# Jiraiya812/Fast-CU-Decision-HEVC

Measured on NVIDIA B200. Metric: cu_decision_ctus_per_s_1080p_all_intra, higher is better.
Workload: dtype int32

## Files before the change

### fast-cu-decision-hevc_b200/csrc/capi.cu

```cuda
#include <cuda_runtime.h>
#include <algorithm>
#include <chrono>
#include <cstdio>
#include <cstdlib>
#include <cstring>
#include "handle.h"
#include "rmd_tc2.cuh"
#include "rmd_tc3.cuh"
#include "tcm_host.h"

using namespace cucd;

static_assert(kPackedCtuBytes == CUCD_PACKED_CTU_BYTES && kPackedU16Off == CUCD_PACKED_U16_OFFSET && kPackedB13Off == CUCD_PACKED_B13_OFFSET,
              "kernel-side packed cost layout must match include/cucudecide.h");

namespace cucd {
std::string g_createError;

bool pin_host_range(cucd_handle* h, const void* ptr, size_t bytes) {
  if (!ptr || !bytes) return false;
  uintptr_t lo = (uintptr_t)ptr, hi = lo + bytes;
  for (const auto& r : h->pins) if (r.first <= lo && hi <= r.second) return true;
  cudaPointerAttributes at;
  if (cudaPointerGetAttributes(&at, ptr) == cudaSuccess && at.type == cudaMemoryTypeHost) {
// ... 24 lines not shown
                              int recStride, uint32_t* out, uint8_t* outPacked, const uint8_t* needed = nullptr) {
  FrameSource fs;
  fs.org = org; fs.rec = rec; fs.orgPicStride = orgPic; fs.recPicStride = recPic; fs.orgStride = orgStride; fs.recStride = recStride;
  fs.W = h->cfg.width; fs.H = h->cfg.height; fs.ctusPerRow = h->ctusPerRow; fs.ctusPerPic = h->ctusPerPic; fs.out = out; fs.outPacked = outPacked; fs.needed = needed;
  return fs;
}
FeaturePlanes make_feature_planes(const cucd_handle* h, const int16_t* org, long long orgPic, int orgStride) {
  FeaturePlanes fp;
  fp.org = org; fp.orgPicStride = orgPic; fp.orgStride = orgStride; fp.W = h->cfg.width; fp.H = h->cfg.height;
  fp.ctusPerRow = h->ctusPerRow; fp.ctusPerPic = h->ctusPerPic; fp.bitDepth = h->cfg.bit_depth;
  return fp;
}

cudaError_t launch_rmd_auto(cucd_handle* h, const FrameSource& fs, int nPics, cudaStream_t st) {
  if (h->useTensor == 1 && h->cfg.bit_depth == 8)
    return launch_rmd_frames_tc2(fs, nPics, h->cfg.strong_intra_smoothing, h->dTc2Tables.p, h->dTc2Tables.p + tc2::kWinTableBytes, h->dHadamard.p, st, &h->launches);
  if (h->useTensor >= 1)
    return launch_rmd_frames_tc3(fs, nPics, h->cfg.bit_depth, h->cfg.strong_intra_smoothing, h->dTc3Tables.p, h->dTc3Tables.p + tc3::kWinTableBytes16,
                                 h->dTc3Tables.p + tc3::kWinTableBytes16 + tc3::kN4TableBytes16, st, &h->launches);
  return launch_rmd_frames(fs, nPics, h->cfg.bit_depth, h->cfg.strong_intra_smoothing, st, &h->launches);
}

bool plane_ok(const void* p, long long picStride, int stride, int width) {
  return ((uintptr_t)p & 15) == 0 && (stride & 7) == 0 && (picStride & 7) == 0 && stride >= width;
}

void fit_batch(cucd_handle* h, int nPics, const uint32_t* hist, int32_t* thr, double* yc ) {
  const int nBlocks = (h->cfg.width / 4) * (h->cfg.height / 4);
  h->pool.run(nPics * 15, [=](int i) {
    const int p = i / 15, f = 1 + i % 15;
    const double y = tcm_fit_one(hist + ((size_t)p * kHistFreqs + f) * kHistBins, nBlocks);
// ... 79 lines not shown
  ok = ok && cudaEventCreate(&h->evK0) == cudaSuccess && cudaEventCreate(&h->evK1) == cudaSuccess;
  ok = ok && cudaEventCreateWithFlags(&h->evMask, cudaEventDisableTiming) == cudaSuccess;
  ok = ok && cudaEventCreateWithFlags(&h->evDevUp, cudaEventDisableTiming) == cudaSuccess && cudaEventCreateWithFlags(&h->evDevDone, cudaEventDisableTiming) == cudaSuccess;
  for (int i = 0; i < cucd_handle::kTimeRing; i++) ok = ok && cudaEventCreate(&h->evRmd0[i]) == cudaSuccess && cudaEventCreate(&h->evRmd1[i]) == cudaSuccess;
  for (FrameSlot& s : h->slots) {
    ok = ok && cudaEventCreateWithFlags(&s.evHist, cudaEventDisableTiming) == cudaSuccess &&
         cudaEventCreateWithFlags(&s.evFork, cudaEventDisableTiming) == cudaSuccess &&
         cudaEventCreateWithFlags(&s.evJoin, cudaEventDisableTiming) == cudaSuccess;
    ok = ok && s.dHist.reserve(P * kHistFreqs * kHistBins) == cudaSuccess && s.dThr.reserve(P * kHistFreqs) == cudaSuccess;
    ok = ok && s.hHist.reserve(P * kHistFreqs * kHistBins) == cudaSuccess && s.hThr.reserve(P * kHistFreqs) == cudaSuccess;
  }
  ok = ok && h->dObf.reserve(P * (size_t)(cfg->width / 4) * (cfg->height / 4)) == cudaSuccess;
  ok = ok && h->dOutlier.reserve(P * (size_t)cfg->width * cfg->height) == cudaSuccess;
  for (int d = 0; d < 4; d++) ok = ok && h->dNum[d].reserve(P * std::max<size_t>(1, h->cuCount[d])) == cudaSuccess && h->dSum[d].reserve(P * std::max<size_t>(1, h->cuCount[d])) == cudaSuccess;
  ok = ok && h->dCtuHad.reserve(P * h->ctusPerPic) == cudaSuccess;
  ok = ok && h->dHadamard.reserve(16384) == cudaSuccess && launch_hadamard_operands(h->dHadamard.p, h->sMain) == cudaSuccess &&
       cudaStreamSynchronize(h->sMain) == cudaSuccess;
  if (ok) {
    std::vector<uint8_t> tab(tc2::kWinTableBytes + tc2::kN4TableBytes);
    tc2::fill_win_tables(tab.data()); tc2::fill_n4_tables(tab.data() + tc2::kWinTableBytes);
    ok = h->dTc2Tables.reserve(tab.size()) == cudaSuccess && cudaMemcpy(h->dTc2Tables.p, tab.data(), tab.size(), cudaMemcpyHostToDevice) == cudaSuccess;
  }
  if (ok) {
    std::vector<uint8_t> tab(tc3::kWinTableBytes16 + tc3::kN4TableBytes16 + tc3::kHadBytes16);
    tc3::fill_win_tables16(tab.data()); tc3::fill_n4_tables16(tab.data() + tc3::kWinTableBytes16);
    tc3::fill_had_tables16(tab.data() + tc3::kWinTableBytes16 + tc3::kN4TableBytes16);
    ok = h->dTc3Tables.reserve(tab.size()) == cudaSuccess && cudaMemcpy(h->dTc3Tables.p, tab.data(), tab.size(), cudaMemcpyHostToDevice) == cudaSuccess;
  }
  h->useTensor = 1;
  { const char* ev = getenv("CUCD_RMD_PATH"); if (ev && !strcmp(ev, "alu")) h->useTensor = 0; }
  if (!ok) {
    const std::string msg = std::string("cucd_create: allocation failed: ") + cudaGetErrorString(cudaGetLastError());
    cucd_destroy(h);
    return fail(nullptr, CUCD_ERR_NOMEM, msg);
  }
  *out = h;
  return CUCD_OK;
}

int cucd_destroy(cucd_handle* h) {
  if (!h) return CUCD_OK;
  cudaSetDevice(h->cfg.device);
  cudaDeviceSynchronize();
  h->pool.stop();
  for (const auto& r : h->pins) cudaHostUnregister((void*)r.first);
  h->dOrg.release(); h->dRec.release(); h->dOrg8.release(); h->dRec8.release(); h->dObf.release(); h->dOutlier.release(); h->dObf8.release(); h->dOutlier8.release();
  h->dCost.release(); h->dCostPacked.release();
  for (FrameSlot& s : h->slots) {
    s.dHist.release(); s.hHist.release(); s.dThr.release(); s.hThr.release();
    if (s.evHist) cudaEventDestroy(s.evHist);
    if (s.evFork) cudaEventDestroy(s.evFork);
    if (s.evJoin) cudaEventDestroy(s.evJoin);
  }
  for (int d = 0; d < 4; d++) { h->dNum[d].release(); h->dSum[d].release(); }
  h->dCtuHad.release(); h->dHadamard.release(); h->dTc2Tables.release();
  h->bOut.release(); h->bStage.release(); h->hStage.release(); h->hStageOut.release(); h->hScratch.release();
  for (auto& r : h->refs) r.buf.release();
  h->dCur.release(); h->dRefPtr.release(); h->dRefStride.release();
  for (int i = 0; i < cucd_handle::kTimeRing; i++) { if (h->evRmd0[i]) cudaEventDestroy(h->evRmd0[i]); if (h->evRmd1[i]) cudaEventDestroy(h->evRmd1[i]); }
  for (int i = 0; i < cucd_handle::kGroups; i++) { if (h->evUpG[i]) cudaEventDestroy(h->evUpG[i]); if (h->evRmdG[i]) cudaEventDestroy(h->evRmdG[i]); }
  h->hDevScratch.release(); h->dDevStage.release();
  if (h->evDevUp) cudaEventDestroy(h->evDevUp);
  if (h->evDevDone) cudaEventDestroy(h->evDevDone);
  h->dNeeded.release();
  if (h->evMask) cudaEventDestroy(h->evMask);
  if (h->evDirect) cudaEventDestroy(h->evDirect);
  if (h->evK0) cudaEventDestroy(h->evK0);
  if (h->evK1) cudaEventDestroy(h->evK1);
  if (h->sUp) cudaStreamDestroy(h->sUp);
  if (h->evUp) cudaEventDestroy(h->evUp);
// ... 389 lines not shown
```

### fast-cu-decision-hevc_b200/csrc/handle.h

```cpp
#pragma once
#include <cuda_runtime.h>
#include <atomic>
#include <condition_variable>
#include <functional>
#include <mutex>
#include <string>
#include <thread>
#include <vector>
#include "../../include/cucudecide.h"
#include "kernels.h"

namespace cucd {

template <class T> struct DevBuf {
  T* p = nullptr; size_t n = 0;
  cudaError_t reserve(size_t count) {
    if (count <= n) return cudaSuccess;
    if (p) cudaFree(p);
    p = nullptr; n = 0;
    cudaError_t e = cudaMalloc(&p, count * sizeof(T));
    if (e == cudaSuccess) n = count;
    return e;
  }
  void release() { if (p) cudaFree(p); p = nullptr; n = 0; }
// ... 95 lines not shown
  long long rmdCalls = 0;
  int launches = 0;
  long long launchTotal = 0;
  std::string err;
  cucd::HostPool pool;
  cucd::FrameSlot slots[2];
  long long begun = 0, ended = 0;
  cucd::DevBuf<int16_t> dOrg, dRec, dObf, dOutlier;
  cucd::DevBuf<uint8_t> dOrg8, dRec8;
  cucd::DevBuf<uint8_t> dObf8, dOutlier8;
  cucd::DevBuf<uint32_t> dCost;
  cucd::DevBuf<uint8_t> dCostPacked;
  cucd::DevBuf<int8_t> dHadamard;
  cucd::DevBuf<uint8_t> dTc3Tables;
  cucd::DevBuf<uint8_t> dTc2Tables;
  int useTensor = 0;
  cucd::DevBuf<int32_t> dNum[4], dSum[4], dCtuHad;
  size_t cuCount[4] = {0, 0, 0, 0};
  bool prune = false; cucd::PruneSwitches sw = {};
  cucd::DevBuf<uint8_t> dNeeded;
  cudaEvent_t evMask = nullptr;
  std::vector<std::pair<uintptr_t, uintptr_t>> pins;
  cucd::DevBuf<uint8_t> bStage; cucd::DevBuf<uint32_t> bOut;
  cucd::PinBuf<uint8_t> hStage, hStageOut, hScratch;
  cudaEvent_t evDirect = nullptr;
  std::vector<int32_t> tmpOffA, tmpOffB;
  std::vector<cucd::RefPlane> refs;
  bool refTableDirty = true;
  cucd::DevBuf<int16_t> dCur; int curStride = 0; bool curSet = false;
  cucd::DevBuf<const int16_t*> dRefPtr; cucd::DevBuf<int32_t> dRefStride;
// ... 27 lines not shown
```

### fast-cu-decision-hevc_b200/csrc/kernels.h

```cpp
#pragma once
#include <cuda_runtime.h>
#include <stdint.h>
#include "rmd_chunk.cuh"

namespace cucd {

constexpr int kHistBins = 4096;
constexpr int kHistFreqs = 16;

cudaError_t launch_rmd_frames(const FrameSource& fs, int nPics, int bitDepth, int strong, cudaStream_t st, int* launches);
cudaError_t configure_rmd_kernels();
cudaError_t configure_rmd_tc2_kernels();
cudaError_t launch_hadamard_operands(int8_t* dst, cudaStream_t st);
cudaError_t launch_rmd_frames_tc2(const FrameSource& fs, int nPics, int strong, const uint8_t* tabWin, const uint8_t* tabN4, const int8_t* hadamard,
                                  cudaStream_t st, int* launches);
int rmd_tc2_smem_bytes();
cudaError_t configure_rmd_tc3_kernels();
cudaError_t launch_rmd_frames_tc3(const FrameSource& fs, int nPics, int bitDepth, int strong, const uint8_t* tabWin16, const uint8_t* tabN416,
                                  const uint8_t* hadamard16, cudaStream_t st, int* launches);
int rmd_tc3_smem_bytes();
cudaError_t launch_rmd_batch_tc2(int log2n, const BatchSource& bs, int strong, const uint8_t* tabWin, const uint8_t* tabN4, const int8_t* hadamard,
                                 cudaStream_t st, int* launches);
cudaError_t launch_rmd_batch(int log2n, const BatchSource& bs, int bitDepth, int strong, cudaStream_t st, int* launches);

struct FeaturePlanes {
  const int16_t* org; long long orgPicStride; int orgStride;
  int W, H, ctusPerRow, ctusPerPic, bitDepth;
};
cudaError_t launch_feature_hist(const FeaturePlanes& fp, int nPics, uint32_t* hist, cudaStream_t st, int* launches);
cudaError_t launch_copy_words(const uint32_t* src, uint32_t* dst, size_t nWords, cudaStream_t st, int* launches);
// ... 63 lines not shown
```

### fast-cu-decision-hevc_b200/csrc/rmd_tc2_kernels.cu

```cuda
#include <cuda_runtime.h>
#include "rmd_tc2.cuh"
#include "rmd_tc_frame.cuh"
#include "satd_tc.cuh"
#include "kernels.h"

namespace cucd {

extern __shared__ __align__(128) unsigned char smem2[];

using namespace tc;
using namespace tc2;
using namespace tcf;

#ifdef CUCD_TC2_TIMING
__device__ long long* g_tc2Dbg = nullptr;
#ifndef CUCD_TC2_STAMP_TID
#define CUCD_TC2_STAMP_TID 0
#endif
#define TC2_STAMP(i) do { if (g_tc2Dbg && threadIdx.x == CUCD_TC2_STAMP_TID) g_tc2Dbg[(size_t)blockIdx.x * 64 + (i)] = clock64(); } while (0)
#define TC2_FINE(i) do { if (g_tc2Dbg && threadIdx.x == CUCD_TC2_STAMP_TID && pass == 0 && (am == 4 || am == -4)) g_tc2Dbg[(size_t)blockIdx.x * 64 + (am == 4 ? 30 : 40) + (i)] = clock64(); } while (0)
#else
#define TC2_STAMP(i) do { } while (0)
#define TC2_FINE(i) do { } while (0)
#endif
#ifdef CUCD_TC2_WARPSKEW
__device__ long long* g_tc2Skew = nullptr;
#define TC2_SKEW(e) do { if (g_tc2Skew && pass == 0 && (am == 4 || (am == 3 && (e) < 2)) && (threadIdx.x & 31) == 0 && threadIdx.x < 128) g_tc2Skew[(size_t)blockIdx.x * 64 + (threadIdx.x >> 5) * 16 + (am == 4 ? (e) : 9 + (e))] = clock64(); } while (0)
#else
#define TC2_SKEW(e) do { } while (0)
#endif

namespace {

struct Tc2Args {
  FrameSource fs;
  BatchSource bs;
  int strong, totalCtus;
  const uint8_t* tabWin; const uint8_t* tabN4; const int8_t* had;
};

constexpr int kIssuerThreads = 32 * kGroups;
constexpr int kCtaThreads = kThreads + kIssuerThreads;
__device__ __forceinline__ void worker_bar() { asm volatile("bar.sync 1, 256;\n" ::: "memory"); }
template <int LOG2N, bool FRAME>
// ... 25 lines not shown
    return;
  }
#pragma unroll
  for (int c = 0; c < C::CTUS; c++) {
    const int cg = unit * C::CTUS + c;
    uint8_t* valid = smem + C::VALID_OFF + c * 256;
    if (ctuX[c] < 0) {
      for (int p = tid; p < C::PUS; p += kThreads) valid[p] = kPuOutside;
      continue;
    }
    const uint8_t* need = ctu_needed<LOG2N>(fs, cg);
    for (int p = tid; p < C::PUS; p += kThreads) valid[p] = pu_state<LOG2N>(fs, need, ctuX[c], ctuY[c], p);
  }
#pragma unroll
  for (int c = 0; c < C::CTUS; c++)
    if (ctuX[c] >= 0) tile_store<Cfg, LOG2N>(tid, fs.W, fs.H, ctuX[c], ctuY[c], tl[c], smem + C::TILE_OFF + c * C::TILE_BYTES);
  worker_bar();
  TC2_STAMP(51);
#pragma unroll
  for (int c = 0; c < C::CTUS; c++)
    if (ctuX[c] >= 0) build_unfiltered<LOG2N>(tid, c, fs.W, fs.H, ctuX[c], ctuY[c], smem + C::TILE_OFF + c * C::TILE_BYTES, smem);
  TC2_STAMP(52);
  if (C::HAS_FILT) {
    worker_bar();
    TC2_STAMP(53);
#pragma unroll
    for (int c = 0; c < C::CTUS; c++)
      if (ctuX[c] >= 0) build_filtered<LOG2N>(tid, c, a.strong, smem);
  }
}

template <int LOG2N, bool FRAME>
__device__ __forceinline__ void tc2_pass(const Tc2Args& a, const int unit, const int pass, const uint32_t tmemBase, uint32_t& ph1, uint32_t& ph2, const Vec16* pre) {
  typedef Cfg<LOG2N> C;
  constexpr int N = C::N, SEG = RowSeg<LOG2N>::value;
  unsigned char* smem = smem2;
  const int tid = threadIdx.x, grp = tid >> 7, rowTid = tid & 127, warp = tid >> 5, lane = tid & 31;
  const Row r = row_map<LOG2N>(tid, pass);
  unsigned char* store = smem + C::STORE_OFF;
  unsigned char* sA1 = smem + C::A1_OFF + grp * 8192;
  unsigned char* sAorg = smem + C::AORG_OFF + grp * 8192;
  uint64_t* mbar1 = reinterpret_cast<uint64_t*>(smem + C::BAR_OFF) + grp;
  uint64_t* mbar2 = mbar1 + kGroups;
  uint64_t* arrA = mbar1 + 2 * kGroups;
  uint64_t* arrB = mbar1 + 3 * kGroups;
  uint32_t* acc = reinterpret_cast<uint32_t*>(smem + C::ACC_OFF);
  const FrameSource& fs = a.fs;
  const int cg = unit * C::CTUS + r.ctu;
  const bool ok = smem[C::VALID_OFF + r.ctu * 256 + (LOG2N == 2 ? 4 * r.pu : r.pu)] == kPuEvaluate;
  const int slot = pu_slot2<LOG2N>(r.ctu, r.pu);

  uint32_t p[16];
  if (ok) {
    uint32_t raw[16];
    if (FRAME) {
      if (pre && pass == 0) {
#pragma unroll
// ... 181 lines not shown
    TC2_SKEW(6);
    if (lateWindow) stage_window(am - 1, angleNext, buf ^ 1);
    if (am > -8) issue_mma1();
    TC2_FINE(7);
    TC2_SKEW(7);
    cost_out(r.o ? 10 - am : 26 + am, !(r.o && am == -8));
    TC2_FINE(8);
    TC2_SKEW(8);
    if (pass == 0) TC2_STAMP(9 + 8 - am);
    angle = angleNext; angleNext = angleNext2;
  }
  (void)angle;
}

template <int LOG2N>
__device__ __forceinline__ void tc2_issue_pass(const Tc2Args& a, const int pass, const uint32_t tmemBase, const int g, uint32_t& phA, uint32_t& phB, uint32_t& phT) {
  typedef Cfg<LOG2N> C;
  unsigned char* smem = smem2;
  uint64_t* bars = reinterpret_cast<uint64_t*>(smem + C::BAR_OFF);
  uint64_t* bar1 = bars + g;
  uint64_t* bar2 = bars + kGroups + g;
  uint64_t* arrA = bars + 2 * kGroups + g;
  uint64_t* arrB = bars + 3 * kGroups + g;
  uint64_t* barT = bars + 4 * kGroups + g;
  const uint32_t uD1 = tmemBase + g * 128, uA2 = uD1, uD2 = uD1 + 64;
  unsigned char* sB1 = smem + C::B1_OFF + g * 2 * C::B1_BYTES;
  const uint32_t idescPred = make_idesc_i8(128, 64, 0, 0), idescHad = make_idesc_i8(128, 64, 0, 1);
  const uint64_t dHad = make_desc(smem_u32(smem + C::HAD_OFF), 1024, 128), dHadNeg = make_desc(smem_u32(smem + C::HAD_OFF + 4096), 1024, 128);
  const uint64_t dAorg = make_desc(smem_u32(smem + C::AORG_OFF + g * 8192), 2048, 128);
  const uint64_t dB1 = make_desc(smem_u32(sB1), 1024, 128), dA1 = make_desc(smem_u32(smem + C::A1_OFF + g * 8192), 2048, 128);
  constexpr uint64_t kStepB = (2 * 1024) >> 4;
  constexpr uint64_t kStepA = (2 * 2048) >> 4;
  const bool lead = elect_one();

// ... 36 lines not shown
  fetch(8, 0);
  mma2();
  mma1(0);
  fetch(7, 1);
#pragma unroll 1
  for (int am = 8; am >= -8; --am) {
    const int buf = (8 - am) & 1;
    mma2();
    if (am > -8) {
      mma1(buf ^ 1);
      if (am > -7) fetch(am - 2, buf);
    }
  }
}

template <int LOG2N, bool FRAME>
__device__ __noinline__ void tc2_body(const Tc2Args& a, const int unit) {
  typedef Cfg<LOG2N> C;
  unsigned char* smem = smem2;
  const int tid = threadIdx.x, warp = tid >> 5;
  const bool worker = tid < kThreads;
  uint32_t* acc = reinterpret_cast<uint32_t*>(smem + C::ACC_OFF);
  if (FRAME && a.fs.needed) {
    const int any = worker ? fork_states<Cfg, LOG2N>(a.fs, unit, a.totalCtus, smem + C::VALID_OFF, tid, kThreads) : 0;
    if (!__syncthreads_or(any)) {
      if (worker) copy_out<Cfg, LOG2N>(a.fs, unit, a.totalCtus, smem + C::VALID_OFF, false, CostRead<LOG2N>{acc}, tid, kThreads);
      return;
    }
    if (worker) worker_bar();
  }
  uint32_t* tmemSlot = reinterpret_cast<uint32_t*>(smem + C::BAR_OFF + 96);
  if (tid == 0) {
    for (int i = 0; i < 5 * kGroups; i++)
      mbar_init(reinterpret_cast<uint64_t*>(smem + C::BAR_OFF) + i, (i >= 2 * kGroups && i < 4 * kGroups) ? 128 : 1);
    asm volatile("fence.mbarrier_init.release.cluster;\n" ::: "memory");
  }
  uint32_t ph1 = 0, ph2 = 0;
  Vec16 pre[8];
  if (worker) {
  TC2_STAMP(0);
  if (warp == 0) tmem_alloc(tmemSlot, 256);
  TC2_STAMP(58);
  const uint4 hadP = reinterpret_cast<const uint4*>(a.had + (LOG2N == 2 ? 8192 : 0))[tid];
  const uint4 hadN = reinterpret_cast<const uint4*>(a.had + (LOG2N == 2 ? 8192 : 0))[tid + 256];
  int ctuX[C::CTUS], ctuY[C::CTUS];
  TileLoad tl[C::CTUS];
  if (FRAME) setup_loads<Cfg, LOG2N>(a.fs, unit, a.totalCtus, tid, ctuX, ctuY, tl, pre);
  TC2_STAMP(59);
  if (LOG2N >= 4) for (int i = tid; i < C::CTUS * C::PUS * kNumModes; i += kThreads) acc[i] = 0;
  reinterpret_cast<int*>(smem + C::DC_OFF)[tid] = 0;
  reinterpret_cast<uint4*>(smem + C::HAD_OFF)[tid] = hadP;
  TC2_STAMP(60);
  reinterpret_cast<uint4*>(smem + C::HAD_OFF)[tid + 256] = hadN;
  worker_bar();
  TC2_STAMP(50);
  tc2_prologue<LOG2N, FRAME>(a, unit, tl, ctuX, ctuY);
  TC2_STAMP(54);
  tc_fence_before();
  fence_async_smem();
  }
  __syncthreads();
  tc_fence_after();
  const uint32_t tmemBase = *tmemSlot;
  TC2_STAMP(1);
  if (worker) {
#pragma unroll 1
    for (int pass = 0; pass < C::PASSES; pass++) tc2_pass<LOG2N, FRAME>(a, unit, pass, tmemBase, ph1, ph2, FRAME ? pre : nullptr);
  } else {
    uint32_t phA = 0, phB = 0, phT = 0;
#pragma unroll 1
    for (int pass = 0; pass < C::PASSES; pass++) tc2_issue_pass<LOG2N>(a, pass, tmemBase, warp - kThreads / 32, phA, phB, phT);
  }
  TC2_STAMP(2);

  tc_fence_before();
  bool mine = true;
  if (FRAME && worker) mine = all_evaluated<Cfg, LOG2N>(smem + C::VALID_OFF, tid, kThreads);
  const bool allEval = __syncthreads_and(mine) && unit * C::CTUS + C::CTUS <= a.totalCtus;
  if (!worker) return;
  if (!FRAME) {
    const BatchSource& bs = a.bs;
    for (int i = tid; i < C::CTUS * C::PUS * kNumModes; i += kThreads) {
      const int pl = i / kNumModes, m = i - pl * kNumModes, idx = unit * C::CTUS * C::PUS + pl;
      if (idx >= bs.count) continue;
      bs.out[(size_t)bs.pus[idx].outIndex * kNumModes + m] = CostRead<LOG2N>{acc}(0, i);
    }
    if (warp == 0) tmem_dealloc(tmemBase, 256);
    return;
  }
  copy_out<Cfg, LOG2N>(a.fs, unit, a.totalCtus, smem + C::VALID_OFF, allEval, CostRead<LOG2N>{acc}, tid, kThreads);
  if (warp == 0) tmem_dealloc(tmemBase, 256);
  TC2_STAMP(3);
#ifdef CUCD_TC2_TIMING
  if (g_tc2Dbg && tid == 0) g_tc2Dbg[(size_t)blockIdx.x * 64 + 4] = LOG2N;
#endif
}

__global__ void __launch_bounds__(kCtaThreads, 2)
rmd_frame_tc2_kernel(const __grid_constant__ Tc2Args a) {
  const FrameBlock fb = frame_block(a.totalCtus, blockIdx.x);
  switch (fb.log2n) {
    case 6: tc2_body<6, true>(a, fb.unit); break;
    case 5: tc2_body<5, true>(a, fb.unit); break;
    case 4: tc2_body<4, true>(a, fb.unit); break;
    case 3: tc2_body<3, true>(a, fb.unit); break;
    default: tc2_body<2, true>(a, fb.unit);
  }
}

template <int LOG2N>
__global__ void __launch_bounds__(kCtaThreads, 2)
rmd_batch_tc2_kernel(const __grid_constant__ Tc2Args a) { tc2_body<LOG2N, false>(a, blockIdx.x); }

template <int LOG2N>
cudaError_t launch_batch_tc2(const Tc2Args& a, int units, cudaStream_t st) {
  rmd_batch_tc2_kernel<LOG2N><<<(units + Cfg<LOG2N>::CTUS - 1) / Cfg<LOG2N>::CTUS, kCtaThreads, Cfg<LOG2N>::TOTAL, st>>>(a);
  return cudaGetLastError();
}

}

int rmd_tc2_smem_bytes() { return kSmemBytes; }

cudaError_t configure_rmd_tc2_kernels() {
  cudaError_t e = cudaFuncSetAttribute(rmd_frame_tc2_kernel, cudaFuncAttributeMaxDynamicSharedMemorySize, kSmemBytes);
  if (e == cudaSuccess) e = cudaFuncSetAttribute(rmd_batch_tc2_kernel<2>, cudaFuncAttributeMaxDynamicSharedMemorySize, Cfg<2>::TOTAL);
  if (e == cudaSuccess) e = cudaFuncSetAttribute(rmd_batch_tc2_kernel<3>, cudaFuncAttributeMaxDynamicSharedMemorySize, Cfg<3>::TOTAL);
  if (e == cudaSuccess) e = cudaFuncSetAttribute(rmd_batch_tc2_kernel<4>, cudaFuncAttributeMaxDynamicSharedMemorySize, Cfg<4>::TOTAL);
  if (e == cudaSuccess) e = cudaFuncSetAttribute(rmd_batch_tc2_kernel<5>, cudaFuncAttributeMaxDynamicSharedMemorySize, Cfg<5>::TOTAL);
  if (e == cudaSuccess) e = cudaFuncSetAttribute(rmd_batch_tc2_kernel<6>, cudaFuncAttributeMaxDynamicSharedMemorySize, Cfg<6>::TOTAL);
  return e;
}

cudaError_t launch_rmd_batch_tc2(int log2n, const BatchSource& bs, int strong, const uint8_t* tabWin, const uint8_t* tabN4, const int8_t* hadamard,
                                 cudaStream_t st, int* launches) {
  if (bs.count <= 0) return cudaSuccess;
  const int n = 1 << log2n, pus = 4096 / (n * n);
  Tc2Args a;
  a.fs = FrameSource{}; a.bs = bs; a.strong = strong; a.totalCtus = (bs.count + pus - 1) / pus; a.tabWin = tabWin; a.tabN4 = tabN4; a.had = hadamard;
  cudaError_t e;
  switch (log2n) {
    case 2: e = launch_batch_tc2<2>(a, a.totalCtus, st); break;
    case 3: e = launch_batch_tc2<3>(a, a.totalCtus, st); break;
    case 4: e = launch_batch_tc2<4>(a, a.totalCtus, st); break;
    case 5: e = launch_batch_tc2<5>(a, a.totalCtus, st); break;
    case 6: e = launch_batch_tc2<6>(a, a.totalCtus, st); break;
    default: return cudaErrorInvalidValue;
  }
  if (e == cudaSuccess && launches) *launches += 1;
  return e;
}

cudaError_t launch_rmd_frames_tc2(const FrameSource& fs, int nPics, int strong, const uint8_t* tabWin, const uint8_t* tabN4, const int8_t* hadamard,
                                  cudaStream_t st, int* launches) {
  const int total = nPics * fs.ctusPerPic;
  if (total <= 0) return cudaSuccess;
  Tc2Args a;
  a.fs = fs; a.bs = BatchSource{}; a.strong = strong; a.totalCtus = total; a.tabWin = tabWin; a.tabN4 = tabN4; a.had = hadamard;
  rmd_frame_tc2_kernel<<<frame_blocks(total), kCtaThreads, kSmemBytes, st>>>(a);
  if (launches) *launches += 1;
  return cudaGetLastError();
}

}
```

### profiles/ubench/rmd_variants.cu

```cuda
#include <cstdio>
#include <cstdlib>
#include <vector>
#ifndef KERNEL
#define KERNEL 2
#endif
#if KERNEL == 2
#include "../../fast-cu-decision-hevc_b200/csrc/rmd_tc2_kernels.cu"
#else
#include "../../fast-cu-decision-hevc_b200/csrc/rmd_tc3_kernels.cu"
#endif

using namespace cucd;
#define CK(x) do { cudaError_t e = (x); if (e != cudaSuccess) { printf("CUDA error %s at %d\n", cudaGetErrorString(e), __LINE__); return 1; } } while (0)
int main(int argc, char** argv) {
  const int W = 1920, H = 1080, P = argc > 1 ? atoi(argv[1]) : 16, reps = argc > 2 ? atoi(argv[2]) : 10, pitch = 1920;
  const int bd = KERNEL == 2 ? 8 : 10;
  const int ctusPerRow = 30, ctusPerPic = 30 * 17, total = P * ctusPerPic;
  std::vector<int16_t> h((size_t)P * pitch * H), hr(h.size());
  srand(1);
  for (int p = 0; p < P; p++)
    for (int y = 0; y < H; y++)
      for (int x = 0; x < W; x++) {
        const unsigned hsh = (unsigned)((y / 8) * 7919 + (x / 8) * 104729 + p * 31) * 2654435761u;
        int v = (int)((hsh >> 24) & 255) * 3 / 5 + 40 + (rand() % 13) - 6;
// ... 15 lines not shown
  {
    std::vector<int8_t> had(16384, 0);
    for (int j = 0; j < 64; j++)
      for (int k = 0; k < 64; k++) {
        const int y = k >> 3, x = k & 7, off = tc2::umma_off64(j, k);
        const int s8 = (__builtin_popcount((j >> 3) & y) + __builtin_popcount((j & 7) & x)) & 1;
        had[off] = (int8_t)(s8 ? -1 : 1); had[4096 + off] = (int8_t)(s8 ? 1 : -1);
        const int q = j >> 4, u = (j >> 2) & 3, v = j & 3, qk = (y >> 2) * 2 + (x >> 2);
        const int s4 = (__builtin_popcount(u & (y & 3)) + __builtin_popcount(v & (x & 3))) & 1;
        const int e = q == qk ? (s4 ? -1 : 1) : 0;
        had[8192 + off] = (int8_t)e; had[12288 + off] = (int8_t)(-e);
      }
    CK(cudaMemcpy(dHad, had.data(), had.size(), cudaMemcpyHostToDevice));
  }
  CK(configure_rmd_tc2_kernels());
  auto launch = [&]() { return launch_rmd_frames_tc2(fs, P, 1, dTab, dTab + tc2::kWinTableBytes, dHad, 0, nullptr); };
#else
  uint8_t* dTab;
  std::vector<uint8_t> tab(tc3::kWinTableBytes16 + tc3::kN4TableBytes16 + tc3::kHadBytes16);
  tc3::fill_win_tables16(tab.data()); tc3::fill_n4_tables16(tab.data() + tc3::kWinTableBytes16); tc3::fill_had_tables16(tab.data() + tc3::kWinTableBytes16 + tc3::kN4TableBytes16);
  CK(cudaMalloc(&dTab, tab.size())); CK(cudaMemcpy(dTab, tab.data(), tab.size(), cudaMemcpyHostToDevice));
  CK(configure_rmd_tc3_kernels());
  auto launch = [&]() { return launch_rmd_frames_tc3(fs, P, bd, 1, dTab, dTab + tc3::kWinTableBytes16, dTab + tc3::kWinTableBytes16 + tc3::kN4TableBytes16, 0, nullptr); };
#endif
  cudaEvent_t e0, e1; cudaEventCreate(&e0); cudaEventCreate(&e1);
  for (int it = 0; it < 3; it++) CK(launch());
  CK(cudaDeviceSynchronize());
  cudaEventRecord(e0);
  for (int it = 0; it < reps; it++) CK(launch());
  cudaEventRecord(e1); CK(cudaDeviceSynchronize());
  float ms; cudaEventElapsedTime(&ms, e0, e1); ms /= reps;
// ... 8 lines not shown
```

### profiles/ubench/tc2_timing.cu

```cuda
#include <cstdio>
#include <cstdlib>
#include <vector>
#include <algorithm>
#include "../../fast-cu-decision-hevc_b200/csrc/rmd_tc2_kernels.cu"

using namespace cucd;
#define CK(x) do { cudaError_t e = (x); if (e != cudaSuccess) { printf("CUDA error %s at %d\n", cudaGetErrorString(e), __LINE__); return 1; } } while (0)
int main(int argc, char** argv) {
  const int W = 1920, H = 1080, P = argc > 1 ? atoi(argv[1]) : 4, pitch = 1920;
  const int ctusPerRow = 30, ctusPerPic = 30 * 17, total = P * ctusPerPic;
  std::vector<int16_t> h((size_t)P * pitch * H);
  srand(1); for (auto& v : h) v = rand() & 255;
  int16_t *dOrg, *dRec; uint32_t* dOut; int8_t* dHad; uint8_t* dTab; long long* dDbg;
  CK(cudaMalloc(&dOrg, h.size() * 2)); CK(cudaMalloc(&dRec, h.size() * 2)); CK(cudaMalloc(&dOut, (size_t)total * 341 * 35 * 4));
  CK(cudaMalloc(&dHad, 16384)); CK(cudaMalloc(&dTab, tc2::kWinTableBytes + tc2::kN4TableBytes));
  CK(cudaMemcpy(dOrg, h.data(), h.size() * 2, cudaMemcpyHostToDevice)); CK(cudaMemcpy(dRec, h.data(), h.size() * 2, cudaMemcpyHostToDevice));
  std::vector<uint8_t> tab(tc2::kWinTableBytes + tc2::kN4TableBytes);
  tc2::fill_win_tables(tab.data()); tc2::fill_n4_tables(tab.data() + tc2::kWinTableBytes);
  CK(cudaMemcpy(dTab, tab.data(), tab.size(), cudaMemcpyHostToDevice));
  {
    std::vector<int8_t> had(16384, 0);
    for (int j = 0; j < 64; j++)
      for (int k = 0; k < 64; k++) {
        const int y = k >> 3, x = k & 7, off = tc2::umma_off64(j, k);
        const int s8 = (__builtin_popcount((j >> 3) & y) + __builtin_popcount((j & 7) & x)) & 1;
        had[off] = (int8_t)(s8 ? -1 : 1); had[4096 + off] = (int8_t)(s8 ? 1 : -1);
        const int q = j >> 4, u = (j >> 2) & 3, v = j & 3, qk = (y >> 2) * 2 + (x >> 2);
        const int s4 = (__builtin_popcount(u & (y & 3)) + __builtin_popcount(v & (x & 3))) & 1;
        const int e = q == qk ? (s4 ? -1 : 1) : 0;
        had[8192 + off] = (int8_t)e; had[12288 + off] = (int8_t)(-e);
      }
    CK(cudaMemcpy(dHad, had.data(), had.size(), cudaMemcpyHostToDevice));
  }
  const int u2 = (total + 1) / 2, u4 = (total + 3) / 4, blocks = 2 * u4 + 3 * u2;
  CK(cudaMalloc(&dDbg, (size_t)blocks * 64 * 8)); CK(cudaMemset(dDbg, 0, (size_t)blocks * 64 * 8));
  CK(cudaMemcpyToSymbol(g_tc2Dbg, &dDbg, sizeof(dDbg)));
  FrameSource fs; fs.org = dOrg; fs.rec = dRec; fs.orgPicStride = (long long)pitch * H; fs.recPicStride = fs.orgPicStride; fs.orgStride = pitch; fs.recStride = pitch;
  fs.W = W; fs.H = H; fs.ctusPerRow = ctusPerRow; fs.ctusPerPic = ctusPerPic; fs.out = dOut; fs.outPacked = nullptr; fs.needed = nullptr;
  CK(configure_rmd_tc2_kernels());
  cudaEvent_t e0, e1; cudaEventCreate(&e0); cudaEventCreate(&e1);
  for (int it = 0; it < 3; it++) {
    cudaEventRecord(e0);
    CK(launch_rmd_frames_tc2(fs, P, 1, dTab, dTab + tc2::kWinTableBytes, dHad, 0, nullptr));
    cudaEventRecord(e1); CK(cudaDeviceSynchronize());
    float ms; cudaEventElapsedTime(&ms, e0, e1); printf("launch %d: %.3f ms (%d CTUs, %.2f M CTU/s)\n", it, ms, total, total / ms / 1e3);
  }
  std::vector<long long> d((size_t)blocks * 64); CK(cudaMemcpy(d.data(), dDbg, d.size() * 8, cudaMemcpyDeviceToHost));
  for (int l = 6; l >= 2; l--) {
    double pro = 0, pass = 0, tail = 0, setup = 0, rounds[17] = {0}; int n = 0;
    for (int b = 0; b < blocks; b++) {
      const long long* t = &d[(size_t)b * 64];
      if (t[4] != l) continue;
      n++; pro += t[1] - t[0]; pass += t[2] - t[1]; tail += t[3] - t[2]; setup += t[8] - t[1];
      for (int r = 0; r < 17; r++) rounds[r] += t[9 + r] - t[8 + r];
    }
    if (!n) continue;
    printf("N=%2d: %5d CTAs  prologue %7.0f  passes %8.0f (first-pass setup %6.0f)  copy-out %6.0f  clk;  rounds am=8..-8:", 1 << l, n, pro / n, pass / n, setup / n, tail / n);
    for (int r = 0; r < 17; r++) printf(" %4.0f", rounds[r] / n);
// ... 24 lines not shown
```

Baseline: 4.210 million.

## Make tc2 frame RMD kernel persistent with atomic work tickets and prefetch

Converts the per-block tc2 frame kernel into a persistent kernel launched with about two CTAs per SM. Each CTA pulls work units through an atomic ticket counter. TMEM allocation, mbarrier init and the Hadamard operand load happen once per CTA (the Hadamard table is reloaded only when the block size changes). The next unit's tile loads are issued before the current unit's copy-out so global loads overlap with output writes. The costs are a memset per launch, extra mbarrier phase bookkeeping across units, and the risk of losing parallelism because of the smaller grid or load imbalance.

Result: slower. 3.145 million, median of 6 (-25.3%).

```diff
diff --git a/fast-cu-decision-hevc_b200/csrc/capi.cu b/fast-cu-decision-hevc_b200/csrc/capi.cu
--- a/fast-cu-decision-hevc_b200/csrc/capi.cu
+++ b/fast-cu-decision-hevc_b200/csrc/capi.cu
@@ -62,7 +62,8 @@
 
 cudaError_t launch_rmd_auto(cucd_handle* h, const FrameSource& fs, int nPics, cudaStream_t st) {
   if (h->useTensor == 1 && h->cfg.bit_depth == 8)
-    return launch_rmd_frames_tc2(fs, nPics, h->cfg.strong_intra_smoothing, h->dTc2Tables.p, h->dTc2Tables.p + tc2::kWinTableBytes, h->dHadamard.p, st, &h->launches);
+    return launch_rmd_frames_tc2(fs, nPics, h->cfg.strong_intra_smoothing, h->dTc2Tables.p, h->dTc2Tables.p + tc2::kWinTableBytes, h->dHadamard.p, h->rmdCtas,
+                                 h->dRmdTickets.p + (h->rmdTicket++ % cucd_handle::kRmdTickets), st, &h->launches);
   if (h->useTensor >= 1)
     return launch_rmd_frames_tc3(fs, nPics, h->cfg.bit_depth, h->cfg.strong_intra_smoothing, h->dTc3Tables.p, h->dTc3Tables.p + tc3::kWinTableBytes16,
                                  h->dTc3Tables.p + tc3::kWinTableBytes16 + tc3::kN4TableBytes16, st, &h->launches);
@@ -172,6 +173,7 @@
   ok = ok && h->dOutlier.reserve(P * (size_t)cfg->width * cfg->height) == cudaSuccess;
   for (int d = 0; d < 4; d++) ok = ok && h->dNum[d].reserve(P * std::max<size_t>(1, h->cuCount[d])) == cudaSuccess && h->dSum[d].reserve(P * std::max<size_t>(1, h->cuCount[d])) == cudaSuccess;
   ok = ok && h->dCtuHad.reserve(P * h->ctusPerPic) == cudaSuccess;
+  ok = ok && h->dRmdTickets.reserve(cucd_handle::kRmdTickets) == cudaSuccess;
   ok = ok && h->dHadamard.reserve(16384) == cudaSuccess && launch_hadamard_operands(h->dHadamard.p, h->sMain) == cudaSuccess &&
        cudaStreamSynchronize(h->sMain) == cudaSuccess;
   if (ok) {
@@ -187,6 +189,8 @@
   }
   h->useTensor = 1;
   { const char* ev = getenv("CUCD_RMD_PATH"); if (ev && !strcmp(ev, "alu")) h->useTensor = 0; }
+  h->rmdCtas = 2 * prop.multiProcessorCount;
+  { const char* ev = getenv("CUCD_RMD_CTAS"); if (ev && atoi(ev) > 0) h->rmdCtas = atoi(ev); }
   if (!ok) {
     const std::string msg = std::string("cucd_create: allocation failed: ") + cudaGetErrorString(cudaGetLastError());
     cucd_destroy(h);
@@ -211,7 +215,7 @@
     if (s.evJoin) cudaEventDestroy(s.evJoin);
   }
   for (int d = 0; d < 4; d++) { h->dNum[d].release(); h->dSum[d].release(); }
-  h->dCtuHad.release(); h->dHadamard.release(); h->dTc2Tables.release();
+  h->dCtuHad.release(); h->dHadamard.release(); h->dTc2Tables.release(); h->dRmdTickets.release();
   h->bOut.release(); h->bStage.release(); h->hStage.release(); h->hStageOut.release(); h->hScratch.release();
   for (auto& r : h->refs) r.buf.release();
   h->dCur.release(); h->dRefPtr.release(); h->dRefStride.release();
diff --git a/fast-cu-decision-hevc_b200/csrc/handle.h b/fast-cu-decision-hevc_b200/csrc/handle.h
--- a/fast-cu-decision-hevc_b200/csrc/handle.h
+++ b/fast-cu-decision-hevc_b200/csrc/handle.h
@@ -133,6 +133,10 @@
   cucd::DevBuf<int8_t> dHadamard;
   cucd::DevBuf<uint8_t> dTc3Tables;
   cucd::DevBuf<uint8_t> dTc2Tables;
+  int rmdCtas = 0;
+  cucd::DevBuf<int> dRmdTickets;
+  unsigned rmdTicket = 0;
+  static constexpr int kRmdTickets = 64;
   int useTensor = 0;
   cucd::DevBuf<int32_t> dNum[4], dSum[4], dCtuHad;
   size_t cuCount[4] = {0, 0, 0, 0};
diff --git a/fast-cu-decision-hevc_b200/csrc/kernels.h b/fast-cu-decision-hevc_b200/csrc/kernels.h
--- a/fast-cu-decision-hevc_b200/csrc/kernels.h
+++ b/fast-cu-decision-hevc_b200/csrc/kernels.h
@@ -13,7 +13,7 @@
 cudaError_t configure_rmd_tc2_kernels();
 cudaError_t launch_hadamard_operands(int8_t* dst, cudaStream_t st);
 cudaError_t launch_rmd_frames_tc2(const FrameSource& fs, int nPics, int strong, const uint8_t* tabWin, const uint8_t* tabN4, const int8_t* hadamard,
-                                  cudaStream_t st, int* launches);
+                                  int ctas, int* ticket, cudaStream_t st, int* launches);
 int rmd_tc2_smem_bytes();
 cudaError_t configure_rmd_tc3_kernels();
 cudaError_t launch_rmd_frames_tc3(const FrameSource& fs, int nPics, int bitDepth, int strong, const uint8_t* tabWin16, const uint8_t* tabN416,
diff --git a/fast-cu-decision-hevc_b200/csrc/rmd_tc2_kernels.cu b/fast-cu-decision-hevc_b200/csrc/rmd_tc2_kernels.cu
--- a/fast-cu-decision-hevc_b200/csrc/rmd_tc2_kernels.cu
+++ b/fast-cu-decision-hevc_b200/csrc/rmd_tc2_kernels.cu
@@ -14,11 +14,12 @@
 
 #ifdef CUCD_TC2_TIMING
 __device__ long long* g_tc2Dbg = nullptr;
+__shared__ int s_tc2Block;
 #ifndef CUCD_TC2_STAMP_TID
 #define CUCD_TC2_STAMP_TID 0
 #endif
-#define TC2_STAMP(i) do { if (g_tc2Dbg && threadIdx.x == CUCD_TC2_STAMP_TID) g_tc2Dbg[(size_t)blockIdx.x * 64 + (i)] = clock64(); } while (0)
-#define TC2_FINE(i) do { if (g_tc2Dbg && threadIdx.x == CUCD_TC2_STAMP_TID && pass == 0 && (am == 4 || am == -4)) g_tc2Dbg[(size_t)blockIdx.x * 64 + (am == 4 ? 30 : 40) + (i)] = clock64(); } while (0)
+#define TC2_STAMP(i) do { if (g_tc2Dbg && threadIdx.x == CUCD_TC2_STAMP_TID) g_tc2Dbg[(size_t)s_tc2Block * 64 + (i)] = clock64(); } while (0)
+#define TC2_FINE(i) do { if (g_tc2Dbg && threadIdx.x == CUCD_TC2_STAMP_TID && pass == 0 && (am == 4 || am == -4)) g_tc2Dbg[(size_t)s_tc2Block * 64 + (am == 4 ? 30 : 40) + (i)] = clock64(); } while (0)
 #else
 #define TC2_STAMP(i) do { } while (0)
 #define TC2_FINE(i) do { } while (0)
@@ -28,6 +29,11 @@
 #define TC2_SKEW(e) do { if (g_tc2Skew && pass == 0 && (am == 4 || (am == 3 && (e) < 2)) && (threadIdx.x & 31) == 0 && threadIdx.x < 128) g_tc2Skew[(size_t)blockIdx.x * 64 + (threadIdx.x >> 5) * 16 + (am == 4 ? (e) : 9 + (e))] = clock64(); } while (0)
 #else
 #define TC2_SKEW(e) do { } while (0)
+#endif
+#ifdef CUCD_V_NO_SETUP_IO
+constexpr bool kKoSetupIo = true;
+#else
+constexpr bool kKoSetupIo = false;
 #endif
 
 namespace {
@@ -83,7 +89,7 @@
   }
 #pragma unroll
   for (int c = 0; c < C::CTUS; c++)
-    if (ctuX[c] >= 0) tile_store<Cfg, LOG2N>(tid, fs.W, fs.H, ctuX[c], ctuY[c], tl[c], smem + C::TILE_OFF + c * C::TILE_BYTES);
+    if (ctuX[c] >= 0 && !kKoSetupIo) tile_store<Cfg, LOG2N>(tid, fs.W, fs.H, ctuX[c], ctuY[c], tl[c], smem + C::TILE_OFF + c * C::TILE_BYTES);
   worker_bar();
   TC2_STAMP(51);
 #pragma unroll
@@ -100,7 +106,7 @@
 }
 
 template <int LOG2N, bool FRAME>
-__device__ __forceinline__ void tc2_pass(const Tc2Args& a, const int unit, const int pass, const uint32_t tmemBase, uint32_t& ph1, uint32_t& ph2, const Vec16* pre) {
+__device__ __forceinline__ void tc2_pass(const Tc2Args& a, const int unit, const int pass, const uint32_t tmemBase, uint64_t* bars, uint32_t& ph1, uint32_t& ph2, const Vec16* pre) {
   typedef Cfg<LOG2N> C;
   constexpr int N = C::N, SEG = RowSeg<LOG2N>::value;
   unsigned char* smem = smem2;
@@ -109,7 +115,7 @@
   unsigned char* store = smem + C::STORE_OFF;
   unsigned char* sA1 = smem + C::A1_OFF + grp * 8192;
   unsigned char* sAorg = smem + C::AORG_OFF + grp * 8192;
-  uint64_t* mbar1 = reinterpret_cast<uint64_t*>(smem + C::BAR_OFF) + grp;
+  uint64_t* mbar1 = bars + grp;
   uint64_t* mbar2 = mbar1 + kGroups;
   uint64_t* arrA = mbar1 + 2 * kGroups;
   uint64_t* arrB = mbar1 + 3 * kGroups;
@@ -321,10 +327,9 @@
 }
 
 template <int LOG2N>
-__device__ __forceinline__ void tc2_issue_pass(const Tc2Args& a, const int pass, const uint32_t tmemBase, const int g, uint32_t& phA, uint32_t& phB, uint32_t& phT) {
+__device__ __forceinline__ void tc2_issue_pass(const Tc2Args& a, const int pass, const uint32_t tmemBase, uint64_t* bars, const int g, uint32_t& phA, uint32_t& phB, uint32_t& phT) {
   typedef Cfg<LOG2N> C;
   unsigned char* smem = smem2;
-  uint64_t* bars = reinterpret_cast<uint64_t*>(smem + C::BAR_OFF);
   uint64_t* bar1 = bars + g;
   uint64_t* bar2 = bars + kGroups + g;
   uint64_t* arrA = bars + 2 * kGroups + g;
@@ -391,103 +396,206 @@
   }
 }
 
-template <int LOG2N, bool FRAME>
+template <int LOG2N>
 __device__ __noinline__ void tc2_body(const Tc2Args& a, const int unit) {
   typedef Cfg<LOG2N> C;
   unsigned char* smem = smem2;
   const int tid = threadIdx.x, warp = tid >> 5;
   const bool worker = tid < kThreads;
   uint32_t* acc = reinterpret_cast<uint32_t*>(smem + C::ACC_OFF);
-  if (FRAME && a.fs.needed) {
-    const int any = worker ? fork_states<Cfg, LOG2N>(a.fs, unit, a.totalCtus, smem + C::VALID_OFF, tid, kThreads) : 0;
-    if (!__syncthreads_or(any)) {
-      if (worker) copy_out<Cfg, LOG2N>(a.fs, unit, a.totalCtus, smem + C::VALID_OFF, false, CostRead<LOG2N>{acc}, tid, kThreads);
-      return;
-    }
-    if (worker) worker_bar();
-  }
+  uint64_t* bars = reinterpret_cast<uint64_t*>(smem + C::BAR_OFF);
   uint32_t* tmemSlot = reinterpret_cast<uint32_t*>(smem + C::BAR_OFF + 96);
   if (tid == 0) {
     for (int i = 0; i < 5 * kGroups; i++)
-      mbar_init(reinterpret_cast<uint64_t*>(smem + C::BAR_OFF) + i, (i >= 2 * kGroups && i < 4 * kGroups) ? 128 : 1);
+      mbar_init(bars + i, (i >= 2 * kGroups && i < 4 * kGroups) ? 128 : 1);
     asm volatile("fence.mbarrier_init.release.cluster;\n" ::: "memory");
   }
   uint32_t ph1 = 0, ph2 = 0;
-  Vec16 pre[8];
   if (worker) {
-  TC2_STAMP(0);
-  if (warp == 0) tmem_alloc(tmemSlot, 256);
-  TC2_STAMP(58);
-  const uint4 hadP = reinterpret_cast<const uint4*>(a.had + (LOG2N == 2 ? 8192 : 0))[tid];
-  const uint4 hadN = reinterpret_cast<const uint4*>(a.had + (LOG2N == 2 ? 8192 : 0))[tid + 256];
-  int ctuX[C::CTUS], ctuY[C::CTUS];
-  TileLoad tl[C::CTUS];
-  if (FRAME) setup_loads<Cfg, LOG2N>(a.fs, unit, a.totalCtus, tid, ctuX, ctuY, tl, pre);
-  TC2_STAMP(59);
-  if (LOG2N >= 4) for (int i = tid; i < C::CTUS * C::PUS * kNumModes; i += kThreads) acc[i] = 0;
-  reinterpret_cast<int*>(smem + C::DC_OFF)[tid] = 0;
-  reinterpret_cast<uint4*>(smem + C::HAD_OFF)[tid] = hadP;
-  TC2_STAMP(60);
-  reinterpret_cast<uint4*>(smem + C::HAD_OFF)[tid + 256] = hadN;
-  worker_bar();
-  TC2_STAMP(50);
-  tc2_prologue<LOG2N, FRAME>(a, unit, tl, ctuX, ctuY);
-  TC2_STAMP(54);
-  tc_fence_before();
-  fence_async_smem();
+    if (warp == 0) tmem_alloc(tmemSlot, 256);
+    const uint4 hadP = reinterpret_cast<const uint4*>(a.had + (LOG2N == 2 ? 8192 : 0))[tid];
+    const uint4 hadN = reinterpret_cast<const uint4*>(a.had + (LOG2N == 2 ? 8192 : 0))[tid + 256];
+    if (LOG2N >= 4) for (int i = tid; i < C::CTUS * C::PUS * kNumModes; i += kThreads) acc[i] = 0;
+    reinterpret_cast<int*>(smem + C::DC_OFF)[tid] = 0;
+    reinterpret_cast<uint4*>(smem + C::HAD_OFF)[tid] = hadP;
+    reinterpret_cast<uint4*>(smem + C::HAD_OFF)[tid + 256] = hadN;
+    worker_bar();
+    tc2_prologue<LOG2N, false>(a, unit, nullptr, nullptr, nullptr);
+    tc_fence_before();
+    fence_async_smem();
   }
   __syncthreads();
   tc_fence_after();
   const uint32_t tmemBase = *tmemSlot;
-  TC2_STAMP(1);
   if (worker) {
 #pragma unroll 1
-    for (int pass = 0; pass < C::PASSES; pass++) tc2_pass<LOG2N, FRAME>(a, unit, pass, tmemBase, ph1, ph2, FRAME ? pre : nullptr);
+    for (int pass = 0; pass < C::PASSES; pass++) tc2_pass<LOG2N, false>(a, unit, pass, tmemBase, bars, ph1, ph2, nullptr);
   } else {
     uint32_t phA = 0, phB = 0, phT = 0;
 #pragma unroll 1
-    for (int pass = 0; pass < C::PASSES; pass++) tc2_issue_pass<LOG2N>(a, pass, tmemBase, warp - kThreads / 32, phA, phB, phT);
-  }
+    for (int pass = 0; pass < C::PASSES; pass++) tc2_issue_pass<LOG2N>(a, pass, tmemBase, bars, warp - kThreads / 32, phA, phB, phT);
+  }
+  tc_fence_before();
+  __syncthreads_and(true);
+  if (!worker) return;
+  const BatchSource& bs = a.bs;
+  for (int i = tid; i < C::CTUS * C::PUS * kNumModes; i += kThreads) {
+    const int pl = i / kNumModes, m = i - pl * kNumModes, idx = unit * C::CTUS * C::PUS + pl;
+    if (idx >= bs.count) continue;
+    bs.out[(size_t)bs.pus[idx].outIndex * kNumModes + m] = CostRead<LOG2N>{acc}(0, i);
+  }
+  if (warp == 0) tmem_dealloc(tmemBase, 256);
+}
+
+constexpr int kFrameBarOff = kSmemBytes;
+constexpr int kFrameSmemBytes = kFrameBarOff + 128;
+__device__ __forceinline__ uint64_t* frame_bars() { return reinterpret_cast<uint64_t*>(smem2 + kFrameBarOff); }
+struct FrameCta {
+  uint32_t passes;
+  uint32_t units;
+  int had;
+  bool pending;
+};
+struct FramePrefetch { int ctuX[4], ctuY[4]; TileLoad tl[4]; Vec16 pre[8]; };
+
+template <int LOG2N>
+__device__ __noinline__ int tc2_frame_unit(const Tc2Args& a, const int b, int* ticket, FrameCta& st, FramePrefetch& pf) {
+  typedef Cfg<LOG2N> C;
+  unsigned char* smem = smem2;
+  const int tid = threadIdx.x, warp = tid >> 5;
+  const bool worker = tid < kThreads;
+  uint32_t* acc = reinterpret_cast<uint32_t*>(smem + C::ACC_OFF);
+  uint64_t* bars = frame_bars();
+  int* nextSlot = reinterpret_cast<int*>(smem + kFrameBarOff + 96) + (st.units & 1u);
+  const FrameSource& fs = a.fs;
+  const int unit = frame_block(a.totalCtus, b).unit;
+  const bool pending = st.pending;
+  st.pending = false;
+  st.units++;
+  if (tid == kThreads) *nextSlot = atomicAdd(ticket, 1) + (int)gridDim.x;
+  TC2_STAMP(0);
+  if (fs.needed) {
+    const int any = worker ? fork_states<Cfg, LOG2N>(fs, unit, a.totalCtus, smem + C::VALID_OFF, tid, kThreads) : 0;
+    if (!__syncthreads_or(any)) {
+      if (worker) copy_out<Cfg, LOG2N>(fs, unit, a.totalCtus, smem + C::VALID_OFF, false, CostRead<LOG2N>{acc}, tid, kThreads);
+      const int next = *nextSlot;
+      if (worker) worker_bar();
+      return next;
+    }
+    if (worker) worker_bar();
+  }
+  const bool newHad = st.had != (LOG2N == 2 ? 1 : 0);
+  Vec16 pre[8];
+  if (worker) {
+    uint4 hadP = make_uint4(0, 0, 0, 0), hadN = hadP;
+    if (newHad) {
+      hadP = reinterpret_cast<const uint4*>(a.had + (LOG2N == 2 ? 8192 : 0))[tid];
+      hadN = reinterpret_cast<const uint4*>(a.had + (LOG2N == 2 ? 8192 : 0))[tid + 256];
+    }
+    int ctuX[C::CTUS], ctuY[C::CTUS];
+    TileLoad tl[C::CTUS];
+    if (kKoSetupIo) {
+      for (int c = 0; c < C::CTUS; c++) {
+        const int cg = unit * C::CTUS + c;
+        ctuX[c] = ctuY[c] = -1;
+        if (cg < a.totalCtus) { const CtuPos q = ctu_pos(fs, cg); ctuX[c] = q.x; ctuY[c] = q.y; }
+      }
+      for (int y = 0; y < 8; y++) pre[y] = Vec16{0u, 0u, 0u, 0u};
+    } else if (pending) {
+#pragma unroll
+      for (int c = 0; c < C::CTUS; c++) { ctuX[c] = pf.ctuX[c]; ctuY[c] = pf.ctuY[c]; tl[c] = pf.tl[c]; }
+#pragma unroll
+      for (int y = 0; y < 8; y++) pre[y] = pf.pre[y];
+    } else setup_loads<Cfg, LOG2N>(fs, unit, a.totalCtus, tid, ctuX, ctuY, tl, pre);
+    TC2_STAMP(59);
+    if (LOG2N >= 4) for (int i = tid; i < C::CTUS * C::PUS * kNumModes; i += kThreads) acc[i] = 0;
+    reinterpret_cast<int*>(smem + C::DC_OFF)[tid] = 0;
+    if (newHad) {
+      reinterpret_cast<uint4*>(smem + C::HAD_OFF)[tid] = hadP;
+      reinterpret_cast<uint4*>(smem + C::HAD_OFF)[tid + 256] = hadN;
+    }
+    TC2_STAMP(60);
+    worker_bar();
+    TC2_STAMP(50);
+    tc2_prologue<LOG2N, true>(a, unit, tl, ctuX, ctuY);
+    TC2_STAMP(54);
+    tc_fence_before();
+    fence_async_smem();
+  }
+  st.had = LOG2N == 2 ? 1 : 0;
+  __syncthreads();
+  tc_fence_after();
+  const uint32_t tmemBase = *reinterpret_cast<const uint32_t*>(smem + kFrameBarOff + 88);
+  TC2_STAMP(1);
+  if (worker) {
+    uint32_t ph1 = st.passes & 1u, ph2 = 0;
+#pragma unroll 1
+    for (int pass = 0; pass < C::PASSES; pass++) tc2_pass<LOG2N, true>(a, unit, pass, tmemBase, bars, ph1, ph2, pre);
+  } else {
+    uint32_t phA = 0, phB = st.passes & 1u, phT = st.passes & 1u;
+#pragma unroll 1
+    for (int pass = 0; pass < C::PASSES; pass++) tc2_issue_pass<LOG2N>(a, pass, tmemBase, bars, warp - kThreads / 32, phA, phB, phT);
+  }
+  st.passes += C::PASSES;
   TC2_STAMP(2);
 
   tc_fence_before();
-  bool mine = true;
-  if (FRAME && worker) mine = all_evaluated<Cfg, LOG2N>(smem + C::VALID_OFF, tid, kThreads);
+  const bool mine = worker ? all_evaluated<Cfg, LOG2N>(smem + C::VALID_OFF, tid, kThreads) : true;
   const bool allEval = __syncthreads_and(mine) && unit * C::CTUS + C::CTUS <= a.totalCtus;
-  if (!worker) return;
-  if (!FRAME) {
-    const BatchSource& bs = a.bs;
-    for (int i = tid; i < C::CTUS * C::PUS * kNumModes; i += kThreads) {
-      const int pl = i / kNumModes, m = i - pl * kNumModes, idx = unit * C::CTUS * C::PUS + pl;
-      if (idx >= bs.count) continue;
-      bs.out[(size_t)bs.pus[idx].outIndex * kNumModes + m] = CostRead<LOG2N>{acc}(0, i);
-    }
-    if (warp == 0) tmem_dealloc(tmemBase, 256);
-    return;
-  }
-  copy_out<Cfg, LOG2N>(a.fs, unit, a.totalCtus, smem + C::VALID_OFF, allEval, CostRead<LOG2N>{acc}, tid, kThreads);
-  if (warp == 0) tmem_dealloc(tmemBase, 256);
-  TC2_STAMP(3);
+  const int next = *nextSlot;
+  if (!worker) return next;
+  if (!kKoSetupIo && next < frame_blocks(a.totalCtus) && frame_block(a.totalCtus, next).log2n == LOG2N) {
+    int ctuX[C::CTUS], ctuY[C::CTUS];
+    TileLoad tl[C::CTUS];
+    Vec16 npre[8];
+    setup_loads<Cfg, LOG2N>(fs, frame_block(a.totalCtus, next).unit, a.totalCtus, tid, ctuX, ctuY, tl, npre);
+    copy_out<Cfg, LOG2N>(fs, unit, a.totalCtus, smem + C::VALID_OFF, allEval, CostRead<LOG2N>{acc}, tid, kThreads);
+#pragma unroll
+    for (int c = 0; c < C::CTUS; c++) { pf.ctuX[c] = ctuX[c]; pf.ctuY[c] = ctuY[c]; pf.tl[c] = tl[c]; }
+#pragma unroll
+    for (int y = 0; y < 8; y++) pf.pre[y] = npre[y];
+    st.pending = true;
+  } else if (!kKoSetupIo) {
+    copy_out<Cfg, LOG2N>(fs, unit, a.totalCtus, smem + C::VALID_OFF, allEval, CostRead<LOG2N>{acc}, tid, kThreads);
+  }
+  worker_bar();
+  return next;
+}
+
+__global__ void __launch_bounds__(kCtaThreads, 2)
+rmd_frame_tc2_kernel(const __grid_constant__ Tc2Args a, int* ticket) {
+  const int tid = threadIdx.x;
+  uint64_t* bars = frame_bars();
+  uint32_t* tmemSlot = reinterpret_cast<uint32_t*>(smem2 + kFrameBarOff + 88);
+  if (tid == 0) {
+    for (int i = 0; i < 5 * kGroups; i++)
+      mbar_init(bars + i, (i >= 2 * kGroups && i < 4 * kGroups) ? 128 : 1);
+    asm volatile("fence.mbarrier_init.release.cluster;\n" ::: "memory");
+  }
+  if (tid < 32) tmem_alloc(tmemSlot, 256);
+  __syncthreads();
+  tc_fence_after();
+  FrameCta st{0u, 0u, -1, false};
+  FramePrefetch pf;
+  const int blocks = frame_blocks(a.totalCtus);
+  for (int b = blockIdx.x; b < blocks;) {
 #ifdef CUCD_TC2_TIMING
-  if (g_tc2Dbg && tid == 0) g_tc2Dbg[(size_t)blockIdx.x * 64 + 4] = LOG2N;
+    if (tid == CUCD_TC2_STAMP_TID) s_tc2Block = b;
 #endif
-}
-
-__global__ void __launch_bounds__(kCtaThreads, 2)
-rmd_frame_tc2_kernel(const __grid_constant__ Tc2Args a) {
-  const FrameBlock fb = frame_block(a.totalCtus, blockIdx.x);
-  switch (fb.log2n) {
-    case 6: tc2_body<6, true>(a, fb.unit); break;
-    case 5: tc2_body<5, true>(a, fb.unit); break;
-    case 4: tc2_body<4, true>(a, fb.unit); break;
-    case 3: tc2_body<3, true>(a, fb.unit); break;
-    default: tc2_body<2, true>(a, fb.unit);
-  }
+    switch (frame_block(a.totalCtus, b).log2n) {
+      case 6: b = tc2_frame_unit<6>(a, b, ticket, st, pf); break;
+      case 5: b = tc2_frame_unit<5>(a, b, ticket, st, pf); break;
+      case 4: b = tc2_frame_unit<4>(a, b, ticket, st, pf); break;
+      case 3: b = tc2_frame_unit<3>(a, b, ticket, st, pf); break;
+      default: b = tc2_frame_unit<2>(a, b, ticket, st, pf);
+    }
+  }
+  if (tid < 32) tmem_dealloc(*tmemSlot, 256);
 }
 
 template <int LOG2N>
 __global__ void __launch_bounds__(kCtaThreads, 2)
-rmd_batch_tc2_kernel(const __grid_constant__ Tc2Args a) { tc2_body<LOG2N, false>(a, blockIdx.x); }
+rmd_batch_tc2_kernel(const __grid_constant__ Tc2Args a) { tc2_body<LOG2N>(a, blockIdx.x); }
 
 template <int LOG2N>
 cudaError_t launch_batch_tc2(const Tc2Args& a, int units, cudaStream_t st) {
@@ -500,7 +608,7 @@
 int rmd_tc2_smem_bytes() { return kSmemBytes; }
 
 cudaError_t configure_rmd_tc2_kernels() {
-  cudaError_t e = cudaFuncSetAttribute(rmd_frame_tc2_kernel, cudaFuncAttributeMaxDynamicSharedMemorySize, kSmemBytes);
+  cudaError_t e = cudaFuncSetAttribute(rmd_frame_tc2_kernel, cudaFuncAttributeMaxDynamicSharedMemorySize, kFrameSmemBytes);
   if (e == cudaSuccess) e = cudaFuncSetAttribute(rmd_batch_tc2_kernel<2>, cudaFuncAttributeMaxDynamicSharedMemorySize, Cfg<2>::TOTAL);
   if (e == cudaSuccess) e = cudaFuncSetAttribute(rmd_batch_tc2_kernel<3>, cudaFuncAttributeMaxDynamicSharedMemorySize, Cfg<3>::TOTAL);
   if (e == cudaSuccess) e = cudaFuncSetAttribute(rmd_batch_tc2_kernel<4>, cudaFuncAttributeMaxDynamicSharedMemorySize, Cfg<4>::TOTAL);
@@ -529,12 +637,15 @@
 }
 
 cudaError_t launch_rmd_frames_tc2(const FrameSource& fs, int nPics, int strong, const uint8_t* tabWin, const uint8_t* tabN4, const int8_t* hadamard,
-                                  cudaStream_t st, int* launches) {
+                                  int ctas, int* ticket, cudaStream_t st, int* launches) {
   const int total = nPics * fs.ctusPerPic;
   if (total <= 0) return cudaSuccess;
+  if (ctas < 1 || !ticket) return cudaErrorInvalidValue;
+  cudaError_t e = cudaMemsetAsync(ticket, 0, sizeof(int), st);
+  if (e != cudaSuccess) return e;
   Tc2Args a;
   a.fs = fs; a.bs = BatchSource{}; a.strong = strong; a.totalCtus = total; a.tabWin = tabWin; a.tabN4 = tabN4; a.had = hadamard;
-  rmd_frame_tc2_kernel<<<frame_blocks(total), kCtaThreads, kSmemBytes, st>>>(a);
+  rmd_frame_tc2_kernel<<<ctas < frame_blocks(total) ? ctas : frame_blocks(total), kCtaThreads, kFrameSmemBytes, st>>>(a, ticket);
   if (launches) *launches += 1;
   return cudaGetLastError();
 }
diff --git a/profiles/ubench/rmd_variants.cu b/profiles/ubench/rmd_variants.cu
--- a/profiles/ubench/rmd_variants.cu
+++ b/profiles/ubench/rmd_variants.cu
@@ -53,7 +53,8 @@
     CK(cudaMemcpy(dHad, had.data(), had.size(), cudaMemcpyHostToDevice));
   }
   CK(configure_rmd_tc2_kernels());
-  auto launch = [&]() { return launch_rmd_frames_tc2(fs, P, 1, dTab, dTab + tc2::kWinTableBytes, dHad, 0, nullptr); };
+  int sms = 0, *dTicket; CK(cudaDeviceGetAttribute(&sms, cudaDevAttrMultiProcessorCount, 0)); CK(cudaMalloc(&dTicket, sizeof(int)));
+  auto launch = [&]() { return launch_rmd_frames_tc2(fs, P, 1, dTab, dTab + tc2::kWinTableBytes, dHad, 2 * sms, dTicket, 0, nullptr); };
 #else
   uint8_t* dTab;
   std::vector<uint8_t> tab(tc3::kWinTableBytes16 + tc3::kN4TableBytes16 + tc3::kHadBytes16);
diff --git a/profiles/ubench/tc2_timing.cu b/profiles/ubench/tc2_timing.cu
--- a/profiles/ubench/tc2_timing.cu
+++ b/profiles/ubench/tc2_timing.cu
@@ -38,10 +38,11 @@
   FrameSource fs; fs.org = dOrg; fs.rec = dRec; fs.orgPicStride = (long long)pitch * H; fs.recPicStride = fs.orgPicStride; fs.orgStride = pitch; fs.recStride = pitch;
   fs.W = W; fs.H = H; fs.ctusPerRow = ctusPerRow; fs.ctusPerPic = ctusPerPic; fs.out = dOut; fs.outPacked = nullptr; fs.needed = nullptr;
   CK(configure_rmd_tc2_kernels());
+  int sms = 0, *dTicket; CK(cudaDeviceGetAttribute(&sms, cudaDevAttrMultiProcessorCount, 0)); CK(cudaMalloc(&dTicket, sizeof(int)));
   cudaEvent_t e0, e1; cudaEventCreate(&e0); cudaEventCreate(&e1);
   for (int it = 0; it < 3; it++) {
     cudaEventRecord(e0);
-    CK(launch_rmd_frames_tc2(fs, P, 1, dTab, dTab + tc2::kWinTableBytes, dHad, 0, nullptr));
+    CK(launch_rmd_frames_tc2(fs, P, 1, dTab, dTab + tc2::kWinTableBytes, dHad, 2 * sms, dTicket, 0, nullptr));
     cudaEventRecord(e1); CK(cudaDeviceSynchronize());
     float ms; cudaEventElapsedTime(&ms, e0, e1); printf("launch %d: %.3f ms (%d CTUs, %.2f M CTU/s)\n", it, ms, total, total / ms / 1e3);
   }
```
